# JiuTongBro/vqnerf_release

Hardware: AMD Instinct MI355X
Metric: rays/sec (render) 800x800, 64+64 samples/ray, NeuS SDF 8x256 + colour 4x256 (higher is better)
Workload: dtype f32; 1 GPU; BASELINE configs[1], nerf/hotdog-shaped NeuS render: one whole 800x800 pin-hole view per rank per step (camera at distance 4, fov 0.6911), n_samples=64, n_importance=64, up_sample_steps=4, sdf 8x256; parallelism=views x1 (no data-path collective)

## Files before the change

vqnerf_release_amd/csrc/mlp_prims.h:

```cpp
#pragma once
#include "common.h"

namespace eng {

enum Act : int { ACT_NONE = 0, ACT_RELU = 1, ACT_SOFTPLUS100 = 2, ACT_SIGMOID = 3 };

__device__ __forceinline__ float fast_exp(float x) { return __builtin_amdgcn_exp2f(x * 1.4426950408889634f); }
__device__ __forceinline__ float fast_log(float x) { return __builtin_amdgcn_logf(x) * 0.6931471805599453f; }
__device__ __forceinline__ float fast_rcp(float x) { return __builtin_amdgcn_rcpf(x); }

template <int ACT>
__device__ __forceinline__ float act_fwd(float x) {
  if (ACT == ACT_RELU) return fmaxf(x, 0.f);
  if (ACT == ACT_SOFTPLUS100) {
    const float t = 100.f * x;
    return t > 20.f ? x : 0.01f * fast_log(1.f + fast_exp(t));
  }
  if (ACT == ACT_SIGMOID) return fast_rcp(1.f + fast_exp(-x));
  return x;
}

template <int ACT>
__device__ __forceinline__ float act_bwd_from_out(float h) {
  if (ACT == ACT_RELU) return h > 0.f ? 1.f : 0.f;
  if (ACT == ACT_SOFTPLUS100) return 1.f - fast_exp(-100.f * h);
  if (ACT == ACT_SIGMOID) return h * (1.f - h);
  return 1.f;
}

struct KSegs {
  int rowA, nA, rowB, nB;
};

template <int NW = 4, class Init, class Epi>
__device__ __forceinline__ void gemm_tiles(const f32x4* __restrict__ lds, const KSegs ks,
                                           const f32x4* __restrict__ w, const int n_out_tiles, const int wave,
                                           const int lane, Init init, Epi epi) {
  const int ng = ks.nA + ks.nB;
  for (int ot = wave; ot < n_out_tiles; ot += NW) {
    f32x16 acc;
    const f32x4* __restrict__ wp = w + (size_t)ot * ng * 64 + lane;
    auto brow = [&](int g) { return ((g < ks.nA) ? (ks.rowA + g) : (ks.rowB + (g - ks.nA))) * 64 + lane; };
    f32x4 a0[4], a1[4], bc, bn;
    auto browc = [&](int g) { return brow(min(g, ng - 1)); };
#pragma unroll
    for (int i = 0; i < 4; ++i) a0[i] = wp[min(i, ng - 1) * 64];
    bc = lds[browc(0)];
    __builtin_amdgcn_s_waitcnt(0x0F70);
    init(ot, acc);
    __builtin_amdgcn_s_setprio(1);
    auto block = [&](const f32x4 (&a)[4], int g0) {
#pragma unroll
      for (int i = 0; i < 4; ++i) {
        bn = lds[browc(g0 + i + 1)];
        if (g0 + i < ng) {
#pragma unroll
          for (int j = 0; j < 4; ++j) acc = __builtin_amdgcn_mfma_f32_32x32x2f32(a[i][j], bc[j], acc, 0, 0, 0);
        }
        bc = bn;
      }
    };
    for (int g = 0; g < ng; g += 8) {
#pragma unroll
      for (int i = 0; i < 4; ++i) a1[i] = wp[min(g + 4 + i, ng - 1) * 64];
      block(a0, g);
#pragma unroll
      for (int i = 0; i < 4; ++i) a0[i] = wp[min(g + 8 + i, ng - 1) * 64];
      block(a1, g + 4);
    }
    __builtin_amdgcn_s_setprio(0);
    epi(ot, acc);
  }
}

template <int NW = 4, int NB = 2, class Aux, class Init, class EpiRq>
__device__ __forceinline__ void gemm_tiles_sw(const f32x4* __restrict__ lds, const KSegs ks, const f32x4* __restrict__ w,
                                              const int n_out_tiles, const int wave, const int lane, Aux aux, Init init, EpiRq epi_rq) {
  const int ng = ks.nA + ks.nB;
  auto brow = [&](int g) { g = min(g, ng - 1); return ((g < ks.nA) ? (ks.rowA + g) : (ks.rowB + (g - ks.nA))) * 64 + lane; };
  for (int base = wave; base < n_out_tiles; base += 2 * NW) {
    f32x16 accA, accB;
    f32x4 a[NB][4], bc, bn;
    auto group = [&](const f32x4& af, f32x16& acc) {
#pragma unroll
      for (int j = 0; j < 4; ++j) acc = __builtin_amdgcn_mfma_f32_32x32x2f32(af[j], bc[j], acc, 0, 0, 0);
    };
    auto block = [&](const f32x4 (&af)[4], int g0, f32x16& acc) {
#pragma unroll
      for (int i = 0; i < 4; ++i) {
        bn = lds[brow(g0 + i + 1)];
        if (g0 + i < ng) group(af[i], acc);
        bc = bn;
      }
    };
    auto fill = [&](const f32x4* __restrict__ wp, f32x4 (&af)[4], int g0) {
#pragma unroll
      for (int i = 0; i < 4; ++i) af[i] = wp[min(g0 + i, ng - 1) * 64];
    };
    auto round = [&](const f32x4* __restrict__ wp, int g, int b_first, f32x16& acc) {
#pragma unroll
      for (int b = 0; b < NB; ++b) {
        if (b < b_first) continue;
        fill(wp, a[(b + NB - 1) % NB], g + 4 * (b + NB - 1));
        block(a[b], g + 4 * b, acc);
      }
    };
    {
      const f32x4* __restrict__ wp = w + (size_t)base * ng * 64 + lane;
#pragma unroll
      for (int b = 0; b < NB - 1; ++b) fill(wp, a[b], 4 * b);
      bc = lds[brow(0)];
      __builtin_amdgcn_s_waitcnt(0x0F70);
      aux(base, 0);
      if (base + NW < n_out_tiles) aux(base + NW, 1);
      init(base, 0, accA);
      __builtin_amdgcn_s_setprio(1);
      for (int g = 0; g < ng; g += 4 * NB) round(wp, g, 0, accA);
      __builtin_amdgcn_s_setprio(0);
    }
    const int otB = base + NW;
    if (otB >= n_out_tiles) {
#pragma unroll
      for (int rq = 0; rq < 4; ++rq) epi_rq(base, 0, rq, accA);
      break;
    }
    {
      const f32x4* __restrict__ wp = w + (size_t)otB * ng * 64 + lane;
#pragma unroll
      for (int b = 0; b < NB - 1; ++b) fill(wp, a[b], 4 * b);
      bc = lds[brow(0)];
      __builtin_amdgcn_s_waitcnt(0x0F70);
      init(otB, 1, accB);
      __builtin_amdgcn_s_setprio(1);
      fill(wp, a[NB - 1], 4 * (NB - 1));
#pragma unroll
      for (int i = 0; i < 4; ++i) {
        bn = lds[brow(i + 1)];
        if (i < ng) group(a[0][i], accB);
        bc = bn;
        epi_rq(base, 0, i, accA);
      }
      round(wp, 0, 1, accB);
      for (int g = 4 * NB; g < ng; g += 4 * NB) round(wp, g, 0, accB);
      __builtin_amdgcn_s_setprio(0);
#pragma unroll
      for (int rq = 0; rq < 4; ++rq) epi_rq(otB, 1, rq, accB);
    }
  }
}

template <int NW = 4, class Init, class Epi>
__device__ __forceinline__ void gemm_tiles_chain(const f32x4* __restrict__ lds, const KSegs ks,
                                                 const f32x4* __restrict__ w, const int n_out_tiles, const int wave,
                                                 const int lane, f32x4 (&pre)[4], const f32x4* __restrict__ next_wp,
                                                 Init init, Epi epi) {
  const int ng = ks.nA + ks.nB;
  for (int ot = wave; ot < n_out_tiles; ot += NW) {
    f32x16 acc;
    const f32x4* __restrict__ wp = w + (size_t)ot * ng * 64 + lane;
    auto brow = [&](int g) { return ((g < ks.nA) ? (ks.rowA + g) : (ks.rowB + (g - ks.nA))) * 64 + lane; };
    const bool first = ot == wave;
    f32x4 a0[4], a1[4], bc, bn;
    auto browc = [&](int g) { return brow(min(g, ng - 1)); };
#pragma unroll
    for (int i = 0; i < 4; ++i) { if (first) a0[i] = pre[i]; else a0[i] = wp[min(i, ng - 1) * 64]; }
    bc = lds[browc(0)];
    __builtin_amdgcn_s_waitcnt(0x0F70);
    init(ot, acc);
    __builtin_amdgcn_s_setprio(1);
    auto block = [&](const f32x4 (&a)[4], int g0) {
#pragma unroll
      for (int i = 0; i < 4; ++i) {
        bn = lds[browc(g0 + i + 1)];
        if (g0 + i < ng) {
#pragma unroll
          for (int j = 0; j < 4; ++j) acc = __builtin_amdgcn_mfma_f32_32x32x2f32(a[i][j], bc[j], acc, 0, 0, 0);
        }
        bc = bn;
      }
    };
    for (int g = 0; g < ng; g += 8) {
#pragma unroll
      for (int i = 0; i < 4; ++i) a1[i] = wp[min(g + 4 + i, ng - 1) * 64];
      block(a0, g);
#pragma unroll
      for (int i = 0; i < 4; ++i) a0[i] = wp[min(g + 8 + i, ng - 1) * 64];
      block(a1, g + 4);
    }
    __builtin_amdgcn_s_setprio(0);
    if (ot + NW >= n_out_tiles && next_wp != nullptr) {
#pragma unroll
      for (int i = 0; i < 4; ++i) pre[i] = next_wp[i * 64];
    }
    epi(ot, acc);
  }
  if (wave >= n_out_tiles && next_wp != nullptr) {
#pragma unroll
    for (int i = 0; i < 4; ++i) pre[i] = next_wp[i * 64];
  }
}

template <int NW = 8, class Init, class EpiRq>
__device__ __forceinline__ void gemm_tiles2(const f32x4* __restrict__ lds, const int img_stride, const KSegs ks,
                                            const f32x4* __restrict__ w, const int n_out_tiles, const int wave,
                                            const int lane, f32x4 (&pre)[4], const bool use_pre,
                                            const f32x4* __restrict__ next_wp, Init init, EpiRq epi_rq) {
  const int ng = ks.nA + ks.nB;
  for (int ot = wave; ot < n_out_tiles; ot += NW) {
    f32x16 acc0, acc1;
    const f32x4* __restrict__ wp = w + (size_t)ot * ng * 64 + lane;
    auto brow = [&](int g) { g = min(g, ng - 1); return ((g < ks.nA) ? (ks.rowA + g) : (ks.rowB + (g - ks.nA))) * 64 + lane; };
    f32x4 a0[4], a1[4], pc, qc, pn, qn;
    const bool first = use_pre && ot == wave;
#pragma unroll
    for (int i = 0; i < 4; ++i) {
      if (first) a0[i] = pre[i]; else a0[i] = wp[min(i, ng - 1) * 64];
    }
    { const int r = brow(0); pc = lds[r]; qc = lds[r + img_stride]; }
    __builtin_amdgcn_s_waitcnt(0x0F70);
    init(ot, 0, acc0);
    init(ot, 1, acc1);
    __builtin_amdgcn_s_setprio(1);
    auto block = [&](const f32x4 (&a)[4], int g0) {
#pragma unroll
      for (int i = 0; i < 4; ++i) {
        { const int r = brow(g0 + i + 1); pn = lds[r]; qn = lds[r + img_stride]; }
        if (g0 + i < ng) {
#pragma unroll
          for (int j = 0; j < 4; ++j) {
            acc0 = __builtin_amdgcn_mfma_f32_32x32x2f32(a[i][j], pc[j], acc0, 0, 0, 0);
            acc1 = __builtin_amdgcn_mfma_f32_32x32x2f32(a[i][j], qc[j], acc1, 0, 0, 0);
          }
        }
        pc = pn; qc = qn;
      }
    };
    if ((ng & 7) == 0) {
      for (int g = 0; g < ng - 8; g += 8) {
#pragma unroll
        for (int i = 0; i < 4; ++i) a1[i] = wp[(g + 4 + i) * 64];
        block(a0, g);
#pragma unroll
        for (int i = 0; i < 4; ++i) a0[i] = wp[(g + 8 + i) * 64];
        block(a1, g + 4);
      }
#pragma unroll
      for (int i = 0; i < 4; ++i) a1[i] = wp[(ng - 4 + i) * 64];
      block(a0, ng - 8);
      if (use_pre && ot + NW >= n_out_tiles && next_wp != nullptr) {
#pragma unroll
        for (int i = 0; i < 4; ++i) pre[i] = next_wp[i * 64];
      }
      f32x4 qt[4];
#pragma unroll
      for (int i = 0; i < 4; ++i) {
        { const int r = brow(ng - 4 + i + 1); pn = lds[r]; qn = lds[r + img_stride]; }
        qt[i] = qc;
#pragma unroll
        for (int j = 0; j < 4; ++j) acc0 = __builtin_amdgcn_mfma_f32_32x32x2f32(a1[i][j], pc[j], acc0, 0, 0, 0);
        pc = pn; qc = qn;
      }
#pragma unroll
      for (int i = 0; i < 4; ++i) {
#pragma unroll
        for (int j = 0; j < 4; ++j) acc1 = __builtin_amdgcn_mfma_f32_32x32x2f32(a1[i][j], qt[i][j], acc1, 0, 0, 0);
        epi_rq(ot, 0, i, acc0);
      }
      __builtin_amdgcn_s_setprio(0);
#pragma unroll
      for (int rq = 0; rq < 4; ++rq) epi_rq(ot, 1, rq, acc1);
      continue;
    }
    for (int g = 0; g < ng; g += 8) {
#pragma unroll
      for (int i = 0; i < 4; ++i) a1[i] = wp[min(g + 4 + i, ng - 1) * 64];
      block(a0, g);
#pragma unroll
      for (int i = 0; i < 4; ++i) a0[i] = wp[min(g + 8 + i, ng - 1) * 64];
      block(a1, g + 4);
    }
    if (use_pre && ot + NW >= n_out_tiles && next_wp != nullptr) {
#pragma unroll
      for (int i = 0; i < 4; ++i) pre[i] = next_wp[i * 64];
    }
#pragma unroll
    for (int rq = 0; rq < 4; ++rq) epi_rq(ot, 0, rq, acc0);
    __builtin_amdgcn_s_setprio(0);
#pragma unroll
    for (int rq = 0; rq < 4; ++rq) epi_rq(ot, 1, rq, acc1);
  }
  if (use_pre && wave >= n_out_tiles && next_wp != nullptr) {
#pragma unroll
    for (int i = 0; i < 4; ++i) pre[i] = next_wp[i * 64];
  }
}

__device__ __forceinline__ f32x4 acc_quad(const f32x16& acc, int rq) {
  return (f32x4){acc[4 * rq + 0], acc[4 * rq + 1], acc[4 * rq + 2], acc[4 * rq + 3]};
}

__device__ __forceinline__ void init_bias(const f32x4* __restrict__ bpack, int ot, int lane, f32x16& acc) {
  const f32x4* b = bpack + ot * 8;
  const bool hi = lane >= 32;
#pragma unroll
  for (int rq = 0; rq < 4; ++rq) {
    const f32x4 v0 = b[rq], v1 = b[4 + rq];
    acc[4 * rq + 0] = hi ? v1[0] : v0[0]; acc[4 * rq + 1] = hi ? v1[1] : v0[1];
    acc[4 * rq + 2] = hi ? v1[2] : v0[2]; acc[4 * rq + 3] = hi ? v1[3] : v0[3];
  }
}

__device__ __forceinline__ void init_zero(f32x16& acc) {
#pragma unroll
  for (int i = 0; i < 16; ++i) acc[i] = 0.f;
}

__device__ __forceinline__ void init_rows(const f32x4* __restrict__ rows , int lane, f32x16& acc) {
#pragma unroll
  for (int rq = 0; rq < 4; ++rq) {
    f32x4 v = rows[rq * 64 + lane];
    acc[4 * rq + 0] = v[0]; acc[4 * rq + 1] = v[1]; acc[4 * rq + 2] = v[2]; acc[4 * rq + 3] = v[3];
  }
}

__device__ __forceinline__ float posenc_feat(int f, float x0, float x1, float x2) {
  if (f < 3) return f == 0 ? x0 : (f == 1 ? x1 : x2);
  const int g = f - 3, k = g / 6, m = g - 6 * k, c = m >= 3 ? m - 3 : m;
  const float xc = c == 0 ? x0 : (c == 1 ? x1 : x2);
  const float arg = xc * (float)(1 << k);
  return m < 3 ? sinf(arg) : cosf(arg);
}
__device__ __forceinline__ float posenc_jac(int f, float x0, float x1, float x2, int* comp) {
  if (f < 3) { *comp = f; return 1.f; }
  const int g = f - 3, k = g / 6, m = g - 6 * k, c = m >= 3 ? m - 3 : m;
  const float xc = c == 0 ? x0 : (c == 1 ? x1 : x2);
  const float fr = (float)(1 << k), arg = xc * fr;
  *comp = c;
  return m < 3 ? fr * cosf(arg) : -fr * sinf(arg);
}

__device__ __forceinline__ int row_feat(int r, int h, int j) { return 32 * (r >> 2) + 2 * (4 * (r & 3) + j) + h; }

template <int NOUT, int NW = 4>
__device__ __forceinline__ void rowdot(const f32x4* __restrict__ lds, int row0, int n_rows,
                                       const f32x4* __restrict__ wimg , float* out_s,
                                       int wave, int lane) {
  constexpr int CH = NOUT == 1 ? 8 : (NOUT <= 2 ? 4 : 3);
  float s[NOUT];
#pragma unroll
  for (int o = 0; o < NOUT; ++o) s[o] = 0.f;
  const int h = lane >> 5;
  for (int r0 = wave; r0 < n_rows; r0 += NW * CH) {
    f32x4 b[CH], wv[CH][NOUT];
#pragma unroll
    for (int c = 0; c < CH; ++c) {
      const int r = min(r0 + NW * c, n_rows - 1);
      b[c] = lds[(row0 + r) * 64 + lane];
#pragma unroll
      for (int o = 0; o < NOUT; ++o) wv[c][o] = wimg[(o * n_rows + r) * 2 + h];
    }
#pragma unroll
    for (int c = 0; c < CH; ++c)
      if (r0 + NW * c < n_rows) {
#pragma unroll
        for (int o = 0; o < NOUT; ++o) {
          s[o] = fmaf(b[c][0], wv[c][o][0], s[o]); s[o] = fmaf(b[c][1], wv[c][o][1], s[o]);
          s[o] = fmaf(b[c][2], wv[c][o][2], s[o]); s[o] = fmaf(b[c][3], wv[c][o][3], s[o]);
        }
      }
  }
#pragma unroll
  for (int o = 0; o < NOUT; ++o) {
    s[o] += __shfl_xor(s[o], 32);
    if (h == 0) out_s[(wave * 32 + (lane & 31)) * NOUT + o] = s[o];
  }
}

}
```

vqnerf_release_amd/csrc/neus_mlp.hip:

```cpp
#include "mlp_prims.h"
#include "vqn_neus_desc.h"
#include <stdlib.h>

using namespace eng;

#ifdef VQN_STAMPS
__device__ unsigned long long g_stamps[8];
#define VQN_STAMP_DECL unsigned long long st_[6] = {0, 0, 0, 0, 0, 0}; unsigned long long st_prev = __builtin_amdgcn_s_memtime(); const unsigned long long st_begin = st_prev;
#define VQN_STAMP(i) { const unsigned long long st_now = __builtin_amdgcn_s_memtime(); st_[i] += st_now - st_prev; st_prev = st_now; }
#define VQN_STAMP_FLUSH if (threadIdx.x == 0) { st_[5] = __builtin_amdgcn_s_memtime() - st_begin; for (int i_ = 0; i_ < 6; ++i_) atomicAdd(&g_stamps[i_], st_[i_]); atomicAdd(&g_stamps[6], 1ull); }
extern "C" int vqn_debug_read_stamps(unsigned long long* out, int reset) {
  if (hipMemcpyFromSymbol(out, HIP_SYMBOL(g_stamps), sizeof(unsigned long long) * 8) != hipSuccess) return -3;
  if (reset) { unsigned long long z[8] = {0, 0, 0, 0, 0, 0, 0, 0}; if (hipMemcpyToSymbol(HIP_SYMBOL(g_stamps), z, sizeof(z)) != hipSuccess) return -3; }
  return 0;
}
#else
#define VQN_STAMP_DECL
#define VQN_STAMP(i)
#define VQN_STAMP_FLUSH
#endif

#ifdef VQN_STAMPS
__device__ unsigned long long g_stamps2[16];
#define FS_DECL unsigned long long fs_[16] = {0, 0, 0, 0, 0, 0, 0, 0, 0, 0, 0, 0, 0, 0, 0, 0}; unsigned long long fs_prev = __builtin_amdgcn_s_memtime(); const unsigned long long fs_begin = fs_prev;
// ... 293 lines not shown
    f32x16 acc0, acc1;
    init_zero(acc0); init_zero(acc1);
    const int g0 = kq * gk, g1 = min(ng, g0 + gk);
    const f32x4* __restrict__ wp = w + (size_t)t * ng * 64 + lane;
    for (int g = g0; g < g1; g += 8) {
      f32x4 a[8], p[8], q[8];
#pragma unroll
      for (int i = 0; i < 8; ++i) {
        const int gg = min(g + i, ng - 1), r = (k_row0 + gg) * 64 + lane;
        a[i] = wp[gg * 64]; p[i] = lds[r]; q[i] = lds[r + IS];
      }
#pragma unroll
      for (int i = 0; i < 8; ++i)
        if (g + i < g1) {
#pragma unroll
          for (int j = 0; j < 4; ++j) {
            acc0 = __builtin_amdgcn_mfma_f32_32x32x2f32(a[i][j], p[i][j], acc0, 0, 0, 0);
            acc1 = __builtin_amdgcn_mfma_f32_32x32x2f32(a[i][j], q[i][j], acc1, 0, 0, 0);
          }
        }
    }
#pragma unroll
    for (int rq = 0; rq < 4; ++rq) {
      lds[(tmp_row0 + wave * 4 + rq) * 64 + lane] = acc_quad(acc0, rq);
      lds[IS + (tmp_row0 + wave * 4 + rq) * 64 + lane] = acc_quad(acc1, rq);
    }
  }
  __syncthreads();
  for (int r = wave; r < 8 * emb_tiles; r += 8) {
    const int im = r / (4 * emb_tiles), er = r - im * 4 * emb_tiles, tt = er >> 2, rq = er & 3;
    f32x4* li = lds + (size_t)im * IS;
    f32x4 sum = li[(tmp_row0 + tt * 4 + rq) * 64 + lane];
    for (int k = 1; k < KS; ++k) sum += li[(tmp_row0 + (k * emb_tiles + tt) * 4 + rq) * 64 + lane];
    if (accumulate) sum += li[(e_row0 + er) * 64 + lane];
    li[(e_row0 + er) * 64 + lane] = sum;
  }
  __syncthreads();
}

struct TrainOut {
  float* E; float* OUTF; float* EXTR;
  float* U[VQN_MAX_SDF_LAYERS]; float* GH[VQN_MAX_SDF_LAYERS]; float* C[VQN_MAX_COL_LAYERS];
  int e_tiles, outf_tiles, extr_tiles;
};

__device__ __forceinline__ void tfmt_store_quad(float* __restrict__ T, const long ptile, const int n_ft, const int ft, const int rq,
                                                const int lane, const f32x4 v) {
  float* base = T + ((ptile * n_ft + ft) * 32 + 8 * rq) * 32 + lane;
#pragma unroll
  for (int j = 0; j < 4; ++j) __builtin_nontemporal_store(v[j], base + 64 * j);
}

template <bool FINE, bool TRAIN = false, bool FOLD = false>
__global__ __launch_bounds__(512, 1) void neus_points2_kernel(
    const SdfDesc sd, const ColDesc cd, const f32x4* __restrict__ wsdf, const f32x4* __restrict__ wcol,
    const float* __restrict__ rays_o, const float* __restrict__ rays_d, const float* __restrict__ zv,
    const float* __restrict__ pts_direct, const float* __restrict__ dirs_direct, const long P, const int S,
    f32x4* __restrict__ scratch, float* __restrict__ out_sdf, float* __restrict__ out_grad,
    float* __restrict__ out_rgb, const TrainOut to) {
  extern __shared__ __attribute__((aligned(16))) f32x4 lds[];
  const int MT = sd.max_tiles;
  const int IMG = E_ROWS + 8 * MT, IS = IMG * 64;
  const int X0 = E_ROWS, Y0 = E_ROWS + 4 * MT;
  Smalls2* sm = reinterpret_cast<Smalls2*>(lds + (size_t)2 * IS);
  const int tid = threadIdx.x, lane = tid & 63, h = lane >> 5, p = lane & 31;
  const int wave = __builtin_amdgcn_readfirstlane(tid >> 6);
  const int img = wave >> 2, w4 = wave & 3;
  f32x4* ldsi = lds + (size_t)img * IS;
  const int n_lin = sd.n_lin;
  const int emb_tiles = (sd.emb_feats + 31) >> 5;
  const long n_tiles = (P + 31) >> 5, n_pairs = (n_tiles + 1) >> 1;
  const size_t per_img = (size_t)(n_lin - 1) * 4 * MT * 64;
#ifdef VQN_DIAG_STASH_ROT
  f32x4* save0 = nullptr;
#else
  f32x4* save0 = FINE ? scratch + (size_t)blockIdx.x * 2 * per_img : nullptr;
#endif
  const int feat_slot = (n_lin - 2) * 4 * MT;
  constexpr bool fold = FOLD;
  static_assert(!FOLD || (FINE && !TRAIN), "the fold is an inference path: the backward and the weight gradients read OUTF");
  f32x4 pre[4];
  f32x4 nopre[4];

  FS_DECL
  for (long pair = blockIdx.x; pair < n_pairs; pair += gridDim.x) {
#ifdef VQN_DIAG_STASH_ROT
    if (FINE) save0 = scratch + ((size_t)((pair / gridDim.x) % VQN_DIAG_STASH_ROT) * gridDim.x + blockIdx.x) * 2 * per_img;
#endif
    FS(12)
    if (tid < 64) {
      const int im = tid >> 5, t = tid & 31;
      long pt = ((2 * pair + im) << 5) + t;
      if (pt >= P) pt = P - 1;
      float x, y, z, dx = 0.f, dy = 0.f, dz = 0.f;
      if (pts_direct != nullptr) {
        x = pts_direct[pt * 3 + 0]; y = pts_direct[pt * 3 + 1]; z = pts_direct[pt * 3 + 2];
        if (FINE) { dx = dirs_direct[pt * 3 + 0]; dy = dirs_direct[pt * 3 + 1]; dz = dirs_direct[pt * 3 + 2]; }
      } else {
        const long ray = pt / S;
        const float tt = zv[pt];
        dx = rays_d[ray * 3 + 0]; dy = rays_d[ray * 3 + 1]; dz = rays_d[ray * 3 + 2];
        x = rays_o[ray * 3 + 0] + __fmul_rn(dx, tt);
        y = rays_o[ray * 3 + 1] + __fmul_rn(dy, tt);
        z = rays_o[ray * 3 + 2] + __fmul_rn(dz, tt);
      }
      sm->pts[im][t * 3 + 0] = x; sm->pts[im][t * 3 + 1] = y; sm->pts[im][t * 3 + 2] = z;
      sm->dirs[im][t * 3 + 0] = dx; sm->dirs[im][t * 3 + 1] = dy; sm->dirs[im][t * 3 + 2] = dz;
    }
    __syncthreads();
    const float xs = sm->pts[img][p * 3 + 0] * sd.scale, ys = sm->pts[img][p * 3 + 1] * sd.scale, zs = sm->pts[img][p * 3 + 2] * sd.scale;
    const long ptile_w = 2 * pair + img;
    for (int r = w4; r < (TRAIN ? 4 * to.e_tiles : sd.emb_rows); r += 4) {
      f32x4 v;
#pragma unroll
      for (int j = 0; j < 4; ++j) {
        const int f = row_feat(r, h, j);
        v[j] = (r < sd.emb_rows && f < sd.emb_feats) ? posenc_feat(f, xs, ys, zs) : 0.f;
      }
      if (r < sd.emb_rows) ldsi[(E0 + r) * 64 + lane] = v;
      if (TRAIN && ptile_w < n_tiles) tfmt_store_quad(to.E, ptile_w, to.e_tiles, r >> 2, r & 3, lane, v);
    }
    __syncthreads();

    FS(0)
    int cur = X0, oth = Y0;
    if (wave < sd.layers[0].n_out_tiles) {
      const f32x4* wp0 = wsdf + sd.layers[0].w_off + (size_t)wave * sd.emb_rows * 64 + lane;
#pragma unroll
      for (int i = 0; i < 4; ++i) pre[i] = wp0[min(i, sd.emb_rows - 1) * 64];
    }
    for (int l = 0; l < n_lin - 1; ++l) {
      const LayerDesc L = sd.layers[l];
      const f32x4* next_wp = nullptr;
      if (l + 1 < n_lin - 1 && wave < sd.layers[l + 1].n_out_tiles)
        next_wp = wsdf + sd.layers[l + 1].w_off + (size_t)wave * (4 * L.n_out_tiles + ((l + 1 == sd.skip) ? sd.emb_rows : 0)) * 64 + lane;
      const KSegs ks = (l == 0) ? KSegs{E0, sd.emb_rows, 0, 0}
                                : KSegs{cur, 4 * sd.layers[l - 1].n_out_tiles, E0, (l == sd.skip) ? sd.emb_rows : 0};
      const int dst = (l == 0) ? X0 : oth;
      const bool do_save = FINE && (l < n_lin - 2);
      const f32x4* bp = wsdf + L.b_off;
      float* const t_u = TRAIN ? to.U[l + 1] : nullptr;
      auto bias_init = [&](int ot, int im, f32x16& acc) { if (im == 0) { FS(2) } init_bias(bp, ot, lane, acc); };
      auto epi_rq = [&](int ot, int im, int rq, const f32x16& acc) {
        if (im == 0 && rq == 0) { FS(1) }
        f32x4* li = lds + (size_t)im * IS;
        f32x4* sv = save0 + (size_t)im * per_img + (size_t)l * 4 * MT * 64;
        f32x4 v = {acc[4 * rq], acc[4 * rq + 1], acc[4 * rq + 2], acc[4 * rq + 3]};
#pragma unroll
        for (int j = 0; j < 4; ++j) v[j] = act_fwd<ACT_SOFTPLUS100>(v[j]);
        li[(dst + ot * 4 + rq) * 64 + lane] = v;
        if (do_save) st_stream(sv + (ot * 4 + rq) * 64 + lane, v);
        if (TRAIN && 2 * pair + im < n_tiles) tfmt_store_quad(t_u, 2 * pair + im, L.n_out_tiles, ot, rq, lane, v);
      };
      gemm_tiles2<8>(lds, IS, ks, wsdf + L.w_off, L.n_out_tiles, wave, lane, pre, true, next_wp, bias_init, epi_rq);
      FS(2)
      __syncthreads();
      FS(3)
      if (l == 0) { cur = X0; oth = Y0; } else { const int t = cur; cur = oth; oth = t; }
    }
    const int hid_rows = 4 * sd.layers[n_lin - 2].n_out_tiles;

    rowdot<1>(ldsi, cur, hid_rows, wsdf + sd.last_w_off, sm->part[img], w4, lane);
    if (FINE && sd.layers[n_lin - 1].n_out_tiles > 0) {
      const LayerDesc L = sd.layers[n_lin - 1];
      const f32x4* bp = fold ? wcol + cd.reserved2 : wsdf + L.b_off;
      gemm_tiles2<8>(lds, IS, KSegs{cur, hid_rows, 0, 0}, fold ? wcol + cd.reserved1 : wsdf + L.w_off,
                     fold ? cd.layers[0].n_out_tiles : L.n_out_tiles, wave, lane, nopre, false, nullptr,
                     [&](int ot, int, f32x16& acc) { init_bias(bp, ot, lane, acc); },
                     [&](int ot, int im, int rq, const f32x16& acc) {
                       f32x4* sv = save0 + (size_t)im * per_img + (size_t)feat_slot * 64;
                       const f32x4 v = {acc[4 * rq], acc[4 * rq + 1], acc[4 * rq + 2], acc[4 * rq + 3]};
                       st_stream(sv + (ot * 4 + rq) * 64 + lane, v);
                       if (TRAIN && 2 * pair + im < n_tiles) {
                         float* base = to.OUTF + (2 * pair + im) * (long)to.outf_tiles * 1024;
#pragma unroll
                         for (int j = 0; j < 4; ++j) {
                           const int f = 32 * ot + 2 * (4 * rq + j) + h + 1;
                           if (f < 32 * to.outf_tiles) __builtin_nontemporal_store(v[j], base + f * 32 + p);
                         }
                       }
                     });
    }
    __syncthreads();
    if (tid < 64) {
      const int im = tid >> 5, t = tid & 31;
      const long pt = ((2 * pair + im) << 5) + t;
      if (pt < P) {
        const float* pr = sm->part[im];
        const float s = ((pr[t] + pr[32 + t]) + (pr[64 + t] + pr[96 + t])) + (sd.last_b_off > 0 ? wsdf[sd.last_b_off][0] : sd.last_bias);
        out_sdf[pt] = s / sd.scale;
      }
      if (TRAIN && 2 * pair + im < n_tiles) {
        float* base = to.OUTF + (2 * pair + im) * (long)to.outf_tiles * 1024;
        const float* pr = sm->part[im];
        base[t] = ((pr[t] + pr[32 + t]) + (pr[64 + t] + pr[96 + t])) + (sd.last_b_off > 0 ? wsdf[sd.last_b_off][0] : sd.last_bias);
        for (int f = 32 * sd.layers[n_lin - 1].n_out_tiles + 1; f < 32 * to.outf_tiles; ++f) base[f * 32 + t] = 0.f;
      }
    }
    if (!FINE) { __syncthreads(); FS(4) continue; }
    FS(4)

    float* const t_gh_top = TRAIN ? to.GH[n_lin - 2] : nullptr;
    for (int r0 = w4; r0 < hid_rows; r0 += 32) {
      f32x4 v[8], wv[8];
#pragma unroll
      for (int c = 0; c < 8; ++c) {
        const int r = min(r0 + 4 * c, hid_rows - 1);
        v[c] = ldsi[(cur + r) * 64 + lane];
        wv[c] = wsdf[sd.last_w_off + r * 2 + h];
      }
#pragma unroll
      for (int c = 0; c < 8; ++c)
        if (r0 + 4 * c < hid_rows) {
#pragma unroll
          for (int j = 0; j < 4; ++j) v[c][j] = wv[c][j] * act_bwd_from_out<ACT_SOFTPLUS100>(v[c][j]);
          ldsi[(cur + r0 + 4 * c) * 64 + lane] = v[c];
          if (TRAIN && ptile_w < n_tiles)
            tfmt_store_quad(t_gh_top, ptile_w, sd.layers[n_lin - 2].n_out_tiles, (r0 + 4 * c) >> 2, (r0 + 4 * c) & 3, lane, v[c]);
        }
    }
    __syncthreads();
    FS(5)
    for (int l = n_lin - 2; l >= 1; --l) {
      const LayerDesc L = sd.layers[l];
      const KSegs ks{cur, 4 * L.n_out_tiles, 0, 0};
      const int dst = oth;
      if (l == sd.skip)
        wte_split_k(lds, IS, cur, 4 * L.n_out_tiles, wsdf + L.wTE_off, emb_tiles, oth, 4 * MT, E0, false, wave, lane);
      f32x4 hv[2][4];
      float* const t_gh = TRAIN ? to.GH[l - 1] : nullptr;
      const int gh_tiles = sd.layers[l - 1].n_out_tiles;
      gemm_tiles2<8>(lds, IS, ks, wsdf + L.wT_off, sd.layers[l - 1].n_out_tiles, wave, lane, nopre, false, nullptr,
                     [&](int ot, int im, f32x16& acc) {
                       if (im == 0) { FS(7) }
                       const f32x4* sv = save0 + (size_t)im * per_img + (size_t)(l - 1) * 4 * MT * 64;
#pragma unroll
                       for (int rq = 0; rq < 4; ++rq) hv[im][rq] = ld_stream(sv + (ot * 4 + rq) * 64 + lane);
                       init_zero(acc);
                     },
                     [&](int ot, int im, int rq, const f32x16& acc) {
                       if (im == 0 && rq == 0) { FS(6) }
                       f32x4* li = lds + (size_t)im * IS;
                       f32x4 v = {acc[4 * rq], acc[4 * rq + 1], acc[4 * rq + 2], acc[4 * rq + 3]};
#pragma unroll
                       for (int j = 0; j < 4; ++j) v[j] *= act_bwd_from_out<ACT_SOFTPLUS100>(hv[im][rq][j]);
                       li[(dst + ot * 4 + rq) * 64 + lane] = v;
                       if (TRAIN && 2 * pair + im < n_tiles) tfmt_store_quad(t_gh, 2 * pair + im, gh_tiles, ot, rq, lane, v);
                     });
      FS(7)
      __syncthreads();
      FS(8)
      const int t = cur; cur = oth; oth = t;
    }
    wte_split_k(lds, IS, cur, 4 * sd.layers[0].n_out_tiles, wsdf + sd.layers[0].wTE_off, emb_tiles, oth, 4 * MT, E0, sd.skip >= 1, wave, lane);
    FS(6)
    if (tid < 192) {
      const int im = tid / 96, r = tid - 96 * im, pp = r & 31, c = r >> 5;
      const float x0 = sm->pts[im][pp * 3 + 0] * sd.scale, x1 = sm->pts[im][pp * 3 + 1] * sd.scale, x2 = sm->pts[im][pp * 3 + 2] * sd.scale;
      const float* ldsf = reinterpret_cast<const float*>(lds + (size_t)im * IS);
      auto G = [&](int f) {
        const int t = f >> 5, fi = f & 31, hh = fi & 1, rr = fi >> 1;
        return ldsf[(((E0 + t * 4 + (rr >> 2)) * 64) + pp + 32 * hh) * 4 + (rr & 3)];
      };
      float g = G(c);
      int cc;
      for (int k = 0; k < sd.multires; ++k) {
        const int fs = 3 + 6 * k + c, fc = fs + 3;
        g = fmaf(G(fs), posenc_jac(fs, x0, x1, x2, &cc), g);
        g = fmaf(G(fc), posenc_jac(fc, x0, x1, x2, &cc), g);
      }
      sm->grad[im][pp * 3 + c] = g;
      const long pt = ((2 * pair + im) << 5) + pp;
      if (pt < P) out_grad[pt * 3 + c] = g;
    }
    __syncthreads();
    FS(9)
    if (cd.n_lin == 0) continue;

    {
      const float px = sm->pts[img][p * 3 + 0], py = sm->pts[img][p * 3 + 1], pz = sm->pts[img][p * 3 + 2];
      const float dx = sm->dirs[img][p * 3 + 0], dy = sm->dirs[img][p * 3 + 1], dz = sm->dirs[img][p * 3 + 2];
      for (int r = w4; r < (TRAIN ? 4 * to.extr_tiles : cd.extra_rows); r += 4) {
        f32x4 v;
#pragma unroll
        for (int j = 0; j < 4; ++j) {
          const int f = row_feat(r, h, j);
          float val = 0.f;
          if (r >= cd.extra_rows) val = 0.f;
          else if (f < 3) val = f == 0 ? px : (f == 1 ? py : pz);
          else if (f < 3 + cd.n_view_feats) val = posenc_feat(f - 3, dx, dy, dz);
          else if (f < cd.extra_feats) val = sm->grad[img][p * 3 + (f - 3 - cd.n_view_feats)];
          v[j] = val;
        }
        if (r < cd.extra_rows) ldsi[(E0 + r) * 64 + lane] = v;
        if (TRAIN && ptile_w < n_tiles) tfmt_store_quad(to.EXTR, ptile_w, to.extr_tiles, r >> 2, r & 3, lane, v);
      }
      const f32x4* sv = save0 + (size_t)img * per_img + (size_t)feat_slot * 64;
      const int feat_rows = 4 * sd.layers[n_lin - 1].n_out_tiles;
      for (int r0 = w4; r0 < (fold ? 0 : feat_rows); r0 += 32) {
        f32x4 v[8];
#pragma unroll
        for (int c = 0; c < 8; ++c) v[c] = ld_stream(sv + min(r0 + 4 * c, feat_rows - 1) * 64 + lane);
#pragma unroll
        for (int c = 0; c < 8; ++c)
          if (r0 + 4 * c < feat_rows) ldsi[(X0 + r0 + 4 * c) * 64 + lane] = v[c];
      }
      __syncthreads();
      FS(10)
      cur = X0; oth = Y0;
      int in_rows = feat_rows;
      if (fold) {
        const LayerDesc L = cd.layers[0];
        const int dst = oth;
        gemm_tiles2<8>(lds, IS, KSegs{E0, cd.extra_rows, 0, 0}, wcol + cd.reserved3, L.n_out_tiles, wave, lane, nopre, false, nullptr,
                       [&](int ot, int im, f32x16& acc) {
                         const f32x4* pp = save0 + (size_t)im * per_img + (size_t)feat_slot * 64 + ot * 256 + lane;
#pragma unroll
                         for (int rq = 0; rq < 4; ++rq) {
                           const f32x4 v = ld_stream(pp + rq * 64);
                           acc[4 * rq + 0] = v[0]; acc[4 * rq + 1] = v[1]; acc[4 * rq + 2] = v[2]; acc[4 * rq + 3] = v[3];
                         }
                       },
                       [&](int ot, int im, int rq, const f32x16& acc) {
                         f32x4* li = lds + (size_t)im * IS;
                         f32x4 v = {acc[4 * rq], acc[4 * rq + 1], acc[4 * rq + 2], acc[4 * rq + 3]};
#pragma unroll
                         for (int j = 0; j < 4; ++j) v[j] = act_fwd<ACT_RELU>(v[j]);
                         li[(dst + ot * 4 + rq) * 64 + lane] = v;
                       });
        __syncthreads();
        const int t = cur; cur = oth; oth = t;
        in_rows = 4 * L.n_out_tiles;
      }
      for (int l = fold ? 1 : 0; l < cd.n_lin - 1; ++l) {
        const LayerDesc L = cd.layers[l];
        const KSegs ks{cur, in_rows, E0, l == 0 ? cd.extra_rows : 0};
        const f32x4* bp = wcol + L.b_off;
        const int dst = oth;
        float* const t_c = TRAIN ? to.C[l + 1] : nullptr;
        gemm_tiles2<8>(lds, IS, ks, wcol + L.w_off, L.n_out_tiles, wave, lane, nopre, false, nullptr,
                       [&](int ot, int, f32x16& acc) { init_bias(bp, ot, lane, acc); },
                       [&](int ot, int im, int rq, const f32x16& acc) {
                         f32x4* li = lds + (size_t)im * IS;
                         f32x4 v = {acc[4 * rq], acc[4 * rq + 1], acc[4 * rq + 2], acc[4 * rq + 3]};
#pragma unroll
                         for (int j = 0; j < 4; ++j) v[j] = act_fwd<ACT_RELU>(v[j]);
                         li[(dst + ot * 4 + rq) * 64 + lane] = v;
                         if (TRAIN && 2 * pair + im < n_tiles) tfmt_store_quad(t_c, 2 * pair + im, L.n_out_tiles, ot, rq, lane, v);
                       });
        __syncthreads();
        const int t = cur; cur = oth; oth = t;
        in_rows = 4 * L.n_out_tiles;
      }
      FS(11)
      rowdot<3>(ldsi, cur, in_rows, wcol + cd.last_w_off, sm->part[img], w4, lane);
      __syncthreads();
      if (tid < 192) {
        const int im = tid / 96, r = tid - 96 * im, pp = r & 31, o = r >> 5;
        const float* pr = sm->part[im];
        float v = ((pr[(0 * 32 + pp) * 3 + o] + pr[(1 * 32 + pp) * 3 + o]) + (pr[(2 * 32 + pp) * 3 + o] + pr[(3 * 32 + pp) * 3 + o])) +
                  (cd.last_b_off > 0 ? wcol[cd.last_b_off][o] : cd.last_bias[o]);
        if (cd.squeeze_out) v = 1.f / (1.f + expf(-v));
        const long pt = ((2 * pair + im) << 5) + pp;
        if (pt < P) out_rgb[pt * 3 + o] = v;
      }
    }
    __syncthreads();
  }
  FS(12)
  FS_FLUSH
}

int check_sdf_desc(const SdfDesc& d) {
  if (d.n_lin < 2 || d.n_lin > VQN_MAX_SDF_LAYERS) return 1;
  if (d.max_tiles < 1 || d.max_tiles > 16) return 2;
  if (d.emb_feats < 3 || d.emb_feats > 64 || d.emb_rows < 1 || d.emb_rows > 8) return 3;
  if (d.skip >= d.n_lin - 1 || d.skip == 0) return 4;
  for (int l = 0; l < d.n_lin; ++l)
    if (d.layers[l].n_out_tiles < 0 || d.layers[l].n_out_tiles > d.max_tiles) return 5;
  if (!(d.scale > 0.f)) return 6;
  return 0;
}

size_t lds_bytes(int MT) { return (size_t)(E_ROWS + 8 * MT) * 1024 + sizeof(Smalls); }
size_t lds_bytes2(int MT) { return (size_t)2 * (E_ROWS + 8 * MT) * 1024 + sizeof(Smalls2); }

bool use_two_images(int MT) {
  static const bool forced32 = getenv("VQN_NEUS_TILE32") != nullptr;
  return !forced32 && MT >= 5 && lds_bytes2(MT) <= 160 * 1024;
}

}

extern "C" int vqn_neus_sdf_points(const int32_t* sdf_desc, const float* wbuf_sdf, const float* rays_o,
                                   const float* rays_d, const float* z, const float* pts, int64_t P, int S,
                                   float* out_sdf, void* stream) {
  VQN_CHECK_ARG(sdf_desc && wbuf_sdf && out_sdf, "sdf_desc, wbuf_sdf, out_sdf must be non-null");
  VQN_CHECK_ARG(P >= 0, "P >= 0");
  if (P == 0) return VQN_OK;
  VQN_CHECK_ARG(pts != nullptr || (rays_o && rays_d && z && S > 0), "either pts or (rays_o, rays_d, z, S) required");
  SdfDesc sd;
  memcpy(&sd, sdf_desc, sizeof(SdfDesc));
  VQN_CHECK_SHAPE(check_sdf_desc(sd) == 0, "invalid SDF network descriptor");
  ColDesc cd;
  memset(&cd, 0, sizeof(cd));
  const long n_tiles = (P + 31) / 32;
  if (use_two_images(sd.max_tiles)) {
    const size_t lds2 = lds_bytes2(sd.max_tiles);
    VQN_HIP(hipFuncSetAttribute((const void*)neus_points2_kernel<false>, hipFuncAttributeMaxDynamicSharedMemorySize, (int)lds2));
    long grid = (long)vqn_num_cus();
    if (grid > (n_tiles + 1) / 2) grid = (n_tiles + 1) / 2;
    hipLaunchKernelGGL(neus_points2_kernel<false>, dim3((unsigned)grid), dim3(512), lds2, (hipStream_t)stream, sd, cd,
                       reinterpret_cast<const f32x4*>(wbuf_sdf), (const f32x4*)nullptr, rays_o, rays_d, z, pts,
                       (const float*)nullptr, (long)P, S, (f32x4*)nullptr, out_sdf, (float*)nullptr, (float*)nullptr, TrainOut{});
    VQN_LAUNCH_CHECK();
    return VQN_OK;
  }
  const size_t lds = lds_bytes(sd.max_tiles);
  VQN_CHECK_SHAPE(lds <= 160 * 1024, "network too wide for LDS");
  if (lds > 64 * 1024)
    VQN_HIP(hipFuncSetAttribute((const void*)neus_points_kernel<false>, hipFuncAttributeMaxDynamicSharedMemorySize, (int)lds));
  long grid = (long)vqn_num_cus() * 2;
  if (grid > n_tiles) grid = n_tiles;
  hipLaunchKernelGGL(neus_points_kernel<false>, dim3((unsigned)grid), dim3(256), lds, (hipStream_t)stream, sd, cd,
                     reinterpret_cast<const f32x4*>(wbuf_sdf), (const f32x4*)nullptr, rays_o, rays_d, z, pts,
                     (const float*)nullptr, (long)P, S, (f32x4*)nullptr, out_sdf, (float*)nullptr, (float*)nullptr);
  VQN_LAUNCH_CHECK();
  return VQN_OK;
}

extern "C" int vqn_neus_train_fwd(const int32_t* sdf_desc, const float* wbuf_sdf, const int32_t* col_desc, const float* wbuf_col,
                                  const float* pts, const float* dirs, int64_t P, void* scratch, int64_t scratch_bytes,
                                  float* const* tensors, int n_tensors, int e_tiles, int outf_tiles, int extr_tiles, float* out_sdf,
                                  float* out_n, float* out_rgb, void* stream) {
  VQN_CHECK_ARG(sdf_desc && wbuf_sdf && col_desc && wbuf_col && pts && dirs && scratch && tensors && out_sdf && out_n && out_rgb, "null pointer");
  VQN_CHECK_ARG(P >= 1, "P >= 1");
  SdfDesc sd;
  ColDesc cd;
  memcpy(&sd, sdf_desc, sizeof(SdfDesc));
  memcpy(&cd, col_desc, sizeof(ColDesc));
  VQN_CHECK_SHAPE(check_sdf_desc(sd) == 0, "invalid SDF network descriptor");
  VQN_CHECK_SHAPE(cd.n_lin >= 2 && cd.n_lin <= VQN_MAX_COL_LAYERS && cd.d_out == 3 && sd.layers[sd.n_lin - 1].n_out_tiles >= 1, "colour net");
  VQN_CHECK_SHAPE(use_two_images(sd.max_tiles), "the training forward kernel is the two-image form only");
  const int nL = sd.n_lin - 1, nC = cd.n_lin - 1;
  VQN_CHECK_ARG(n_tensors == 3 + 2 * nL + nC, "tensors: [E, OUTF, EXTR, U_1..U_nL, GH_0..GH_{nL-1}, C_1..C_nC]");
  VQN_CHECK_SHAPE(e_tiles * 4 >= sd.emb_rows && e_tiles <= 2 && extr_tiles * 4 >= cd.extra_rows && extr_tiles <= 2 &&
                  outf_tiles >= sd.layers[sd.n_lin - 1].n_out_tiles && 32 * outf_tiles >= 32 * sd.layers[sd.n_lin - 1].n_out_tiles + 1, "tile counts");
  TrainOut to;
  memset(&to, 0, sizeof(to));
  for (int i = 0; i < n_tensors; ++i) VQN_CHECK_ARG(tensors[i] != nullptr, "null tensor pointer");
  to.E = tensors[0]; to.OUTF = tensors[1]; to.EXTR = tensors[2];
  for (int l = 1; l <= nL; ++l) to.U[l] = tensors[3 + (l - 1)];
  for (int l = 0; l < nL; ++l) to.GH[l] = tensors[3 + nL + l];
  for (int l = 1; l <= nC; ++l) to.C[l] = tensors[3 + 2 * nL + (l - 1)];
  to.e_tiles = e_tiles; to.outf_tiles = outf_tiles; to.extr_tiles = extr_tiles;
  const long n_tiles = (P + 31) / 32;
  const int64_t per_wg = (int64_t)(sd.n_lin - 1) * 4 * sd.max_tiles * 1024;
  const size_t lds2 = lds_bytes2(sd.max_tiles);
  VQN_HIP(hipFuncSetAttribute((const void*)neus_points2_kernel<true, true>, hipFuncAttributeMaxDynamicSharedMemorySize, (int)lds2));
  long grid = (long)vqn_num_cus();
  if (grid > (n_tiles + 1) / 2) grid = (n_tiles + 1) / 2;
  if ((int64_t)grid * 2 * per_wg > scratch_bytes) grid = (long)(scratch_bytes / (2 * per_wg));
  VQN_CHECK_ARG(grid >= 1, "scratch too small (see vqn_neus_fine_scratch_bytes)");
  hipLaunchKernelGGL((neus_points2_kernel<true, true>), dim3((unsigned)grid), dim3(512), lds2, (hipStream_t)stream, sd, cd,
                     reinterpret_cast<const f32x4*>(wbuf_sdf), reinterpret_cast<const f32x4*>(wbuf_col), (const float*)nullptr,
                     (const float*)nullptr, (const float*)nullptr, pts, dirs, (long)P, 1, reinterpret_cast<f32x4*>(scratch), out_sdf, out_n,
                     out_rgb, to);
  VQN_LAUNCH_CHECK();
  return VQN_OK;
}

extern "C" int64_t vqn_neus_fine_scratch_bytes(const int32_t* sdf_desc) {
  if (!sdf_desc) return -1;
  SdfDesc sd;
  memcpy(&sd, sdf_desc, sizeof(SdfDesc));
  const int emb_rows = sd.emb_rows;
  if (emb_rows >= 1 && emb_rows <= 12) sd.emb_rows = 1;
  if (check_sdf_desc(sd) != 0) return -2;
#ifdef VQN_DIAG_STASH_ROT
  return (int64_t)VQN_DIAG_STASH_ROT * vqn_num_cus() * 2 * (int64_t)(sd.n_lin - 1) * 4 * sd.max_tiles * 1024;
#else
  return (int64_t)vqn_num_cus() * 2 * (int64_t)(sd.n_lin - 1) * 4 * sd.max_tiles * 1024;
#endif
}

extern "C" int vqn_neus_fine_points(const int32_t* sdf_desc, const float* wbuf_sdf, const int32_t* col_desc,
                                    const float* wbuf_col, const float* rays_o, const float* rays_d, const float* z,
                                    const float* pts, const float* dirs, int64_t P, int S, void* scratch,
                                    int64_t scratch_bytes, float* out_sdf, float* out_grad, float* out_rgb,
                                    void* stream) {
  VQN_CHECK_ARG(sdf_desc && wbuf_sdf && col_desc && wbuf_col, "descriptors and weight packs must be non-null");
  VQN_CHECK_ARG(out_sdf && out_grad && scratch, "out_sdf, out_grad and scratch must be non-null");
  VQN_CHECK_ARG(P >= 0, "P >= 0");
// ... 54 lines not shown
```

Baseline: 280,000 rays/s.

## Balance ragged output tiles across waves and peel K remainder in MFMA GEMM

Adds gemm_tiles2u, a variant of the wave-tiled MFMA GEMM that handles a ragged final round of output tiles. Some waves compute a single image instead of both, so the leftover tile-pairs are spread over more waves. It also peels the K-group remainder into a leading partial block instead of clamping loads, and interleaves the tail MFMAs of the second image with the first image's epilogue. The aim is to cut idle waves and wasted clamped MFMAs in the SDF and colour MLP layers. It costs extra code size and register pressure, and the pre-fetch of the next layer's weights is skipped for single-image waves.

```diff
diff --git a/vqnerf_release_amd/csrc/mlp_prims.h b/vqnerf_release_amd/csrc/mlp_prims.h
--- a/vqnerf_release_amd/csrc/mlp_prims.h
+++ b/vqnerf_release_amd/csrc/mlp_prims.h
@@ -1,5 +1,6 @@
 #pragma once
 #include "common.h"
+#include <type_traits>
 
 namespace eng {
 
@@ -295,6 +296,181 @@
   }
 }
 
+__device__ __forceinline__ int gemm_ragged_splits(const int r) { return min(r & 3, 4 - (r & 3)); }
+
+template <int NW = 8, class Init, class EpiRq>
+__device__ __forceinline__ void gemm_tiles2u(const f32x4* __restrict__ lds, const int img_stride, const KSegs ks,
+                                            const f32x4* __restrict__ w, const int n_out_tiles, const int wave,
+                                            const int lane, f32x4 (&pre)[4], const bool use_pre,
+                                            const f32x4* __restrict__ next_wp, Init init, EpiRq epi_rq) {
+  const int ng = ks.nA + ks.nB;
+  const int rem = n_out_tiles % NW;
+  const int ns = (NW == 8) ? gemm_ragged_splits(rem) : 0;
+  const bool single0 = wave >= rem - ns && wave < rem;
+  const bool single1 = wave >= NW - ns;
+  for (int ot = wave; ot < n_out_tiles - ns; ot += NW) {
+    f32x16 acc0, acc1;
+    const f32x4* __restrict__ wp = w + (size_t)ot * ng * 64 + lane;
+    auto brow = [&](int g) { g = min(g, ng - 1); return ((g < ks.nA) ? (ks.rowA + g) : (ks.rowB + (g - ks.nA))) * 64 + lane; };
+    f32x4 a0[4], a1[4], pc, qc, pn, qn;
+    const bool first = use_pre && ot == wave;
+#pragma unroll
+    for (int i = 0; i < 4; ++i) {
+      if (first) a0[i] = pre[i]; else a0[i] = wp[min(i, ng - 1) * 64];
+    }
+    { const int r = brow(0); pc = lds[r]; qc = lds[r + img_stride]; }
+    __builtin_amdgcn_s_waitcnt(0x0F70);
+    init(ot, 0, acc0);
+    init(ot, 1, acc1);
+    __builtin_amdgcn_s_setprio(1);
+    auto block = [&](const f32x4 (&a)[4], int g0) {
+#pragma unroll
+      for (int i = 0; i < 4; ++i) {
+        { const int r = brow(g0 + i + 1); pn = lds[r]; qn = lds[r + img_stride]; }
+        if (g0 + i < ng) {
+#pragma unroll
+          for (int j = 0; j < 4; ++j) {
+            acc0 = __builtin_amdgcn_mfma_f32_32x32x2f32(a[i][j], pc[j], acc0, 0, 0, 0);
+            acc1 = __builtin_amdgcn_mfma_f32_32x32x2f32(a[i][j], qc[j], acc1, 0, 0, 0);
+          }
+        }
+        pc = pn; qc = qn;
+      }
+    };
+    auto lead_block = [&](const f32x4 (&a)[4], int g0, int n) {
+#pragma unroll
+      for (int i = 0; i < 4; ++i) {
+        if (i < n) {
+          { const int r = brow(g0 + i + 1); pn = lds[r]; qn = lds[r + img_stride]; }
+#pragma unroll
+          for (int j = 0; j < 4; ++j) {
+            acc0 = __builtin_amdgcn_mfma_f32_32x32x2f32(a[i][j], pc[j], acc0, 0, 0, 0);
+            acc1 = __builtin_amdgcn_mfma_f32_32x32x2f32(a[i][j], qc[j], acc1, 0, 0, 0);
+          }
+          pc = pn; qc = qn;
+        }
+      }
+    };
+    if (ng >= 8) {
+      const int lead = ng & 7;
+      if (lead != 0) {
+        const int n0 = min(lead, 4);
+#pragma unroll
+        for (int i = 0; i < 4; ++i) a1[i] = wp[(n0 + i) * 64];
+        lead_block(a0, 0, n0);
+        if (lead > 4) {
+#pragma unroll
+          for (int i = 0; i < 4; ++i) a0[i] = wp[(lead + i) * 64];
+          lead_block(a1, 4, lead - 4);
+        } else {
+#pragma unroll
+          for (int i = 0; i < 4; ++i) a0[i] = a1[i];
+        }
+      }
+      for (int g = lead; g < ng - 8; g += 8) {
+#pragma unroll
+        for (int i = 0; i < 4; ++i) a1[i] = wp[(g + 4 + i) * 64];
+        block(a0, g);
+#pragma unroll
+        for (int i = 0; i < 4; ++i) a0[i] = wp[(g + 8 + i) * 64];
+        block(a1, g + 4);
+      }
+#pragma unroll
+      for (int i = 0; i < 4; ++i) a1[i] = wp[(ng - 4 + i) * 64];
+      block(a0, ng - 8);
+      if (use_pre && !single0 && !single1 && ot + NW >= n_out_tiles && next_wp != nullptr) {
+#pragma unroll
+        for (int i = 0; i < 4; ++i) pre[i] = next_wp[i * 64];
+      }
+      f32x4 qt[4];
+#pragma unroll
+      for (int i = 0; i < 4; ++i) {
+        { const int r = brow(ng - 4 + i + 1); pn = lds[r]; qn = lds[r + img_stride]; }
+        qt[i] = qc;
+#pragma unroll
+        for (int j = 0; j < 4; ++j) acc0 = __builtin_amdgcn_mfma_f32_32x32x2f32(a1[i][j], pc[j], acc0, 0, 0, 0);
+        pc = pn; qc = qn;
+      }
+#pragma unroll
+      for (int i = 0; i < 4; ++i) {
+#pragma unroll
+        for (int j = 0; j < 4; ++j) acc1 = __builtin_amdgcn_mfma_f32_32x32x2f32(a1[i][j], qt[i][j], acc1, 0, 0, 0);
+        epi_rq(ot, 0, i, acc0);
+      }
+      __builtin_amdgcn_s_setprio(0);
+#pragma unroll
+      for (int rq = 0; rq < 4; ++rq) epi_rq(ot, 1, rq, acc1);
+      continue;
+    }
+    for (int g = 0; g < ng; g += 8) {
+#pragma unroll
+      for (int i = 0; i < 4; ++i) a1[i] = wp[min(g + 4 + i, ng - 1) * 64];
+      block(a0, g);
+#pragma unroll
+      for (int i = 0; i < 4; ++i) a0[i] = wp[min(g + 8 + i, ng - 1) * 64];
+      block(a1, g + 4);
+    }
+    if (use_pre && !single0 && !single1 && ot + NW >= n_out_tiles && next_wp != nullptr) {
+#pragma unroll
+      for (int i = 0; i < 4; ++i) pre[i] = next_wp[i * 64];
+    }
+#pragma unroll
+    for (int rq = 0; rq < 4; ++rq) epi_rq(ot, 0, rq, acc0);
+    __builtin_amdgcn_s_setprio(0);
+#pragma unroll
+    for (int rq = 0; rq < 4; ++rq) epi_rq(ot, 1, rq, acc1);
+  }
+  auto one = [&](const int ot, auto im_c) {
+    constexpr int IM = decltype(im_c)::value;
+    f32x16 acc;
+    const f32x4* __restrict__ wp = w + (size_t)ot * ng * 64 + lane;
+    auto brow = [&](int g) { g = min(g, ng - 1); return ((g < ks.nA) ? (ks.rowA + g) : (ks.rowB + (g - ks.nA))) * 64 + lane; };
+    const f32x4* __restrict__ li = lds + (IM ? img_stride : 0);
+    f32x4 a0[4], a1[4], bc, bn;
+    const bool first = use_pre && ot == wave;
+#pragma unroll
+    for (int i = 0; i < 4; ++i) {
+      if (first) a0[i] = pre[i]; else a0[i] = wp[min(i, ng - 1) * 64];
+    }
+    bc = li[brow(0)];
+    __builtin_amdgcn_s_waitcnt(0x0F70);
+    init(ot, IM, acc);
+    __builtin_amdgcn_s_setprio(1);
+    auto block = [&](const f32x4 (&a)[4], int g0) {
+#pragma unroll
+      for (int i = 0; i < 4; ++i) {
+        bn = li[brow(g0 + i + 1)];
+        if (g0 + i < ng) {
+#pragma unroll
+          for (int j = 0; j < 4; ++j) acc = __builtin_amdgcn_mfma_f32_32x32x2f32(a[i][j], bc[j], acc, 0, 0, 0);
+        }
+        bc = bn;
+      }
+    };
+    for (int g = 0; g < ng; g += 8) {
+#pragma unroll
+      for (int i = 0; i < 4; ++i) a1[i] = wp[min(g + 4 + i, ng - 1) * 64];
+      block(a0, g);
+#pragma unroll
+      for (int i = 0; i < 4; ++i) a0[i] = wp[min(g + 8 + i, ng - 1) * 64];
+      block(a1, g + 4);
+    }
+    __builtin_amdgcn_s_setprio(0);
+    if (use_pre && next_wp != nullptr) {
+#pragma unroll
+      for (int i = 0; i < 4; ++i) pre[i] = next_wp[i * 64];
+    }
+#pragma unroll
+    for (int rq = 0; rq < 4; ++rq) epi_rq(ot, IM, rq, acc);
+  };
+  if (single0) one(n_out_tiles - rem + wave, std::integral_constant<int, 0>{});
+  else if (single1) one(n_out_tiles - NW + wave, std::integral_constant<int, 1>{});
+  if (use_pre && !single0 && !single1 && wave >= n_out_tiles && next_wp != nullptr) {
+#pragma unroll
+    for (int i = 0; i < 4; ++i) pre[i] = next_wp[i * 64];
+  }
+}
+
 __device__ __forceinline__ f32x4 acc_quad(const f32x16& acc, int rq) {
   return (f32x4){acc[4 * rq + 0], acc[4 * rq + 1], acc[4 * rq + 2], acc[4 * rq + 3]};
 }
diff --git a/vqnerf_release_amd/csrc/neus_mlp.hip b/vqnerf_release_amd/csrc/neus_mlp.hip
--- a/vqnerf_release_amd/csrc/neus_mlp.hip
+++ b/vqnerf_release_amd/csrc/neus_mlp.hip
@@ -469,7 +469,7 @@
         if (do_save) st_stream(sv + (ot * 4 + rq) * 64 + lane, v);
         if (TRAIN && 2 * pair + im < n_tiles) tfmt_store_quad(t_u, 2 * pair + im, L.n_out_tiles, ot, rq, lane, v);
       };
-      gemm_tiles2<8>(lds, IS, ks, wsdf + L.w_off, L.n_out_tiles, wave, lane, pre, true, next_wp, bias_init, epi_rq);
+      gemm_tiles2u<8>(lds, IS, ks, wsdf + L.w_off, L.n_out_tiles, wave, lane, pre, true, next_wp, bias_init, epi_rq);
       FS(2)
       __syncthreads();
       FS(3)
@@ -481,7 +481,7 @@
     if (FINE && sd.layers[n_lin - 1].n_out_tiles > 0) {
       const LayerDesc L = sd.layers[n_lin - 1];
       const f32x4* bp = fold ? wcol + cd.reserved2 : wsdf + L.b_off;
-      gemm_tiles2<8>(lds, IS, KSegs{cur, hid_rows, 0, 0}, fold ? wcol + cd.reserved1 : wsdf + L.w_off,
+      gemm_tiles2u<8>(lds, IS, KSegs{cur, hid_rows, 0, 0}, fold ? wcol + cd.reserved1 : wsdf + L.w_off,
                      fold ? cd.layers[0].n_out_tiles : L.n_out_tiles, wave, lane, nopre, false, nullptr,
                      [&](int ot, int, f32x16& acc) { init_bias(bp, ot, lane, acc); },
                      [&](int ot, int im, int rq, const f32x16& acc) {
@@ -547,7 +547,7 @@
       f32x4 hv[2][4];
       float* const t_gh = TRAIN ? to.GH[l - 1] : nullptr;
       const int gh_tiles = sd.layers[l - 1].n_out_tiles;
-      gemm_tiles2<8>(lds, IS, ks, wsdf + L.wT_off, sd.layers[l - 1].n_out_tiles, wave, lane, nopre, false, nullptr,
+      gemm_tiles2u<8>(lds, IS, ks, wsdf + L.wT_off, sd.layers[l - 1].n_out_tiles, wave, lane, nopre, false, nullptr,
                      [&](int ot, int im, f32x16& acc) {
                        if (im == 0) { FS(7) }
                        const f32x4* sv = save0 + (size_t)im * per_img + (size_t)(l - 1) * 4 * MT * 64;
@@ -629,7 +629,7 @@
       if (fold) {
         const LayerDesc L = cd.layers[0];
         const int dst = oth;
-        gemm_tiles2<8>(lds, IS, KSegs{E0, cd.extra_rows, 0, 0}, wcol + cd.reserved3, L.n_out_tiles, wave, lane, nopre, false, nullptr,
+        gemm_tiles2u<8>(lds, IS, KSegs{E0, cd.extra_rows, 0, 0}, wcol + cd.reserved3, L.n_out_tiles, wave, lane, nopre, false, nullptr,
                        [&](int ot, int im, f32x16& acc) {
                          const f32x4* pp = save0 + (size_t)im * per_img + (size_t)feat_slot * 64 + ot * 256 + lane;
 #pragma unroll
@@ -655,7 +655,7 @@
         const f32x4* bp = wcol + L.b_off;
         const int dst = oth;
         float* const t_c = TRAIN ? to.C[l + 1] : nullptr;
-        gemm_tiles2<8>(lds, IS, ks, wcol + L.w_off, L.n_out_tiles, wave, lane, nopre, false, nullptr,
+        gemm_tiles2u<8>(lds, IS, ks, wcol + L.w_off, L.n_out_tiles, wave, lane, nopre, false, nullptr,
                        [&](int ot, int, f32x16& acc) { init_bias(bp, ot, lane, acc); },
                        [&](int ot, int im, int rq, const f32x16& acc) {
                          f32x4* li = lds + (size_t)im * IS;
```

Result: slower. 271,400 rays/s (-3.1%).
